# Vahe1994/AQLM

Measured on AMD Instinct MI355X. Metric: QuantizedLinear 1x16g8 matvec algorithmic GB/s (bs=1, Llama-3-8B shapes 4096->4096/11008), higher is better.
Workload: dtype f16; 1 GPU; decode step = 32 blocks x {4096->4096, 4096->11008} 1x16g8 matvec, bs=1, 64 distinct layers (own codes + codebook), 564 MB algorithmic bytes/step, hipGraph replay; scheme=1x16g8, batch=1, kernels=prepacked slice-bucketed gemv (layers of >= 0.5 M codes: both shapes), parallelism=single GPU, packed_bytes=1190264832, canonical_code_bytes=494927872

## Files before the change

aqlm_amd/_native.py:

```python
from __future__ import annotations

import ctypes
import os

_HERE = os.path.dirname(os.path.abspath(__file__))
LIB_PATH = os.environ.get("AQLM_AMD_HIP_LIB") or os.path.join(_HERE, "libaqlm_hip.so")
ABI_VERSION = 9

F16, BF16 = 0, 1
F32 = 2
E_INVALID, E_UNSUPPORTED = -1, -2
MAX_GEMV_BATCH = 8
OP_GEMM_1X16_MFMA = 1
OP_GEMV_1X16_PACKED = 3
OP_GEMV_8X8_LUT = 4
OP_GEMM_KX8_MFMA = 6
OP_GEMV_1X16_G16_PACKED = 5

MAX_SEGMENTS = 4
MAX_ROUTED_PAIRS = 64
MAX_ROUTED_EXPERTS = 256
ROUTED_ENTRY_WORDS = 4
MAX_GROUPED_PAIRS = 1 << 18
GROUPED_TILE_PAIRS = (16, 32, 64, 128)
# ... 219 lines not shown
        raise ImportError(f"{LIB_PATH}: ABI version {v}, expected {ABI_VERSION}; rebuild it")
    return lib


lib = _load()


def last_error() -> str:
    return (lib.aqlm_hip_last_error() or b"").decode("utf-8", "replace")


def check(rc: int, what: str = "") -> None:
    if rc == 0:
        return
    msg = last_error() or what
    if rc == E_UNSUPPORTED:
        raise NotImplementedError(msg)
    if rc == E_INVALID:
        raise ValueError(msg)
    raise AqlmHipError(f"HIP error {rc}: {msg}")


def set_tuning(key: str, value: int) -> None:
    check(lib.aqlm_hip_set_tuning(key.encode(), int(value)), "set_tuning")


def get_tuning(key: str) -> int:
    v = _ci(0)
    check(lib.aqlm_hip_get_tuning(key.encode(), ctypes.byref(v)), "get_tuning")
    return v.value


CAPTURE_OVERLAP_FIELDS = ("seen", "relaxed", "kept_conflict", "kept_window", "runs_broken", "api_failures",
                          "merged", "merge_refused", "nodes_added", "folded")


def capture_overlap_stats(reset: bool = False) -> dict:
    out = (ctypes.c_uint64 * len(CAPTURE_OVERLAP_FIELDS))()
    check(lib.aqlm_hip_capture_overlap_stats_ex(out, len(out)), "capture_overlap_stats")
    if reset:
        check(lib.aqlm_hip_capture_overlap_stats_ex(None, 0), "capture_overlap_stats")
    return dict(zip(CAPTURE_OVERLAP_FIELDS, (int(v) for v in out)))


def packed_image(desc: "PackedDesc", rows: int = 1, dtype: int = F16):
    lds, win = _sz(0), ctypes.c_uint32(0)
    check(lib.aqlm_hip_gemv_1x16_packed_image(ctypes.byref(desc), int(rows), int(dtype), 0, ctypes.byref(lds), ctypes.byref(win), None),
          "packed_image")
    return int(lds.value), int(win.value)


def packed_image_blocks_per_cu(desc: "PackedDesc", rows: int = 1, dtype: int = F16, probe_lds_bytes: int = 0) -> int:
    n = _ci(0)
    check(lib.aqlm_hip_gemv_1x16_packed_image(ctypes.byref(desc), int(rows), int(dtype), int(probe_lds_bytes), None, None, ctypes.byref(n)),
          "packed_image")
    return n.value


def packed_chain_plan(desc: "PackedDesc", next_desc=None, rows: int = 1, dtype: int = F16):
    kept, waves, lds = _ci(0), _ci(0), _sz(0)
    check(lib.aqlm_hip_gemv_1x16_packed_chain_plan(ctypes.byref(desc), int(rows), int(dtype), None if next_desc is None else ctypes.byref(next_desc),
                                                   ctypes.byref(kept), ctypes.byref(waves), ctypes.byref(lds)), "packed_chain_plan")
    return bool(kept.value), int(waves.value), int(lds.value)
```

aqlm_amd/csrc/api.hip:

```cpp
#include <stdarg.h>
#include <string.h>

#include <algorithm>
#include <map>
#include <mutex>
#include <utility>

#include "aqlm_common.h"

namespace aqlm {

static thread_local char g_err[512] = "";

void set_last_error(const char* fmt, ...) {
  va_list ap;
  va_start(ap, fmt);
  vsnprintf(g_err, sizeof(g_err), fmt, ap);
  va_end(ap);
}

int check_hip(hipError_t e, const char* what) {
  if (e == hipSuccess) return 0;
  set_last_error("%s: %s (%d)", what, hipGetErrorString(e), (int)e);
  return (int)e;
// ... 23 lines not shown
static int* tuning_slot(const char* key) {
  Tuning& t = tuning();
  if (!key) return nullptr;
  if (!strcmp(key, "gemv_rows_per_wave")) return &t.gemv_rows_per_wave;
  if (!strcmp(key, "gemv1x16_aux")) return &t.gemv1x16_aux;
  if (!strcmp(key, "gemv1x16_prefetch_cb")) return &t.gemv1x16_prefetch_cb;
  if (!strcmp(key, "kx8_replicas")) return &t.kx8_replicas;
  if (!strcmp(key, "gemm_variant")) return &t.gemm_variant;
  if (!strcmp(key, "kx8_mfma_min_rows")) return &t.kx8_mfma_min_rows;
  if (!strcmp(key, "kx8_xres")) return &t.kx8_xres;
  if (!strcmp(key, "kx8_xres_phased")) return &t.kx8_xres_phased;
  if (!strcmp(key, "kx8_phase_tpb")) return &t.kx8_phase_tpb;
  if (!strcmp(key, "kx8_phase_quads")) return &t.kx8_phase_quads;
  if (!strcmp(key, "kx8_multi_xres_min_rows")) return &t.kx8_multi_xres_min_rows;
  if (!strcmp(key, "kx8_ksplit")) return &t.kx8_ksplit;
  if (!strcmp(key, "kx8_rt")) return &t.kx8_rt;
  if (!strcmp(key, "scan_max_rows")) return &t.scan_max_rows;
  if (!strcmp(key, "scan_prefetch")) return &t.scan_prefetch;
  if (!strcmp(key, "gemm_debug")) return &t.gemm_debug;
  if (!strcmp(key, "gemm_store_nt")) return &t.gemm_store_nt;
  if (!strcmp(key, "force_generic")) return &t.force_generic;
  if (!strcmp(key, "packed_waves")) return &t.packed_waves;
  if (!strcmp(key, "packed_fused_finalize")) return &t.packed_fused_finalize;
  if (!strcmp(key, "packed_prefetch")) return &t.packed_prefetch;
  if (!strcmp(key, "packed_arrange")) return &t.packed_arrange;
  if (!strcmp(key, "packed_xcopies")) return &t.packed_xcopies;
  if (!strcmp(key, "packed_entry_bytes")) return &t.packed_entry_bytes;
  if (!strcmp(key, "packed_debug")) return &t.packed_debug;
  if (!strcmp(key, "packed_fill_rotate")) return &t.packed_fill_rotate;
  if (!strcmp(key, "packed_compact_window")) return &t.packed_compact_window;
  if (!strcmp(key, "packed_capture_window")) return &t.packed_capture_window;
  if (!strcmp(key, "packed_capture_min_run")) return &t.packed_capture_min_run;
  if (!strcmp(key, "packed_capture_merge")) return &t.packed_capture_merge;
  if (!strcmp(key, "packed_group_fold")) return &t.packed_group_fold;
  if (!strcmp(key, "packed_pipe")) return &t.packed_pipe;
  if (!strcmp(key, "packed_prefetch_waves")) return &t.packed_prefetch_waves;
  if (!strcmp(key, "packed_dequant_by_xcd")) return &t.packed_dequant_by_xcd;
  if (!strcmp(key, "lut_waves")) return &t.lut_waves;
  return nullptr;
}

namespace {
struct CaptureOverlapState {
  std::mutex mu;
  capture_overlap::Planner planner;
  uint64_t stats[10] = {0, 0, 0, 0, 0, 0, 0, 0, 0, 0};
  bool off = false;
};
CaptureOverlapState& capture_state() {
  static CaptureOverlapState s;
  return s;
}
hipError_t set_capture_deps(hipStream_t stream, const std::vector<capture_overlap::NodeId>& nodes) {
  static_assert(sizeof(hipGraphNode_t) == sizeof(capture_overlap::NodeId), "a graph node handle is carried as a 64-bit id");
  std::vector<hipGraphNode_t> d;
  for (capture_overlap::NodeId n : nodes) d.push_back(reinterpret_cast<hipGraphNode_t>(static_cast<uintptr_t>(n)));
  return hipStreamUpdateCaptureDependencies(stream, d.empty() ? nullptr : d.data(), d.size(), hipStreamSetCaptureDependencies);
}
bool same_nodes(const std::vector<capture_overlap::NodeId>& a, const std::vector<capture_overlap::NodeId>& b) {
  return a.size() == b.size() && std::is_permutation(a.begin(), a.end(), b.begin());
}
bool read_capture(hipStream_t stream, bool& capturing, unsigned long long& id, std::vector<capture_overlap::NodeId>& deps, hipError_t& err) {
  hipStreamCaptureStatus st = hipStreamCaptureStatusNone;
  const hipGraphNode_t* d = nullptr;
  size_t n = 0;
  hipGraph_t graph = nullptr;
  err = hipStreamGetCaptureInfo_v2(stream, &st, &id, &graph, &d, &n);
  if (err != hipSuccess) return false;
  capturing = st == hipStreamCaptureStatusActive;
  deps.clear();
  if (capturing)
    for (size_t i = 0; i < n; ++i) deps.push_back(static_cast<capture_overlap::NodeId>(reinterpret_cast<uintptr_t>(d[i])));
  return true;
}
}

void CaptureRelax::fail(const char* what, hipError_t e) {
  (void)hipGetLastError();
  CaptureOverlapState& s = capture_state();
  s.off = true;
  ++s.stats[5];
  set_last_error("capture overlap switched off for this process: %s: %s (%d)", what, hipGetErrorString(e), (int)e);
}

CaptureRelax::CaptureRelax(hipStream_t stream) : stream_(stream) {
  if (!stream) return;
  CaptureOverlapState& s = capture_state();
  {
    std::lock_guard<std::mutex> lock(s.mu);
    if (s.off) return;
  }
  bool capturing = false;
  hipError_t err = hipSuccess;
  if (!read_capture(stream, capturing, id_, before_, err)) {
    std::lock_guard<std::mutex> lock(s.mu);
    fail("hipStreamGetCaptureInfo_v2", err);
    return;
  }
  if (!capturing) return;
  const int window = tuning().packed_capture_window;
  std::lock_guard<std::mutex> lock(s.mu);
  ++s.stats[0];
  ++s.stats[8];
  if (window <= 1 && tuning().packed_capture_merge <= 1) ++s.stats[3];
  else active_ = true;
}

void CaptureRelax::apply_plan() {
  CaptureOverlapState& s = capture_state();
  ++s.stats[plan_.kind == capture_overlap::kBroken ? 4 : (int)plan_.kind];
  if (plan_.kind == capture_overlap::kBroken || same_nodes(plan_.deps, before_)) return;
  const hipError_t e = set_capture_deps(stream_, plan_.deps);
  if (e == hipSuccess) {
    changed_ = true;
    return;
  }
  fail("hipStreamUpdateCaptureDependencies", e);
  s.planner.run(id_).reset();
  active_ = false;
}

int CaptureRelax::begin(uint64_t key, const void* member, size_t member_bytes) {
  if (!active_ || begun_) return 0;
  begun_ = true;
  const int merge = std::min(std::max(tuning().packed_capture_merge, 1), capture_overlap::kMaxMerge);
  if (merge > 1 && key != 0 && member) {
    key_ = key;
    member_.assign(static_cast<const unsigned char*>(member), static_cast<const unsigned char*>(member) + member_bytes);
  }
  CaptureOverlapState& s = capture_state();
  std::lock_guard<std::mutex> lock(s.mu);
  plan_ = s.planner.run(id_).plan(before_.data(), before_.size(), fp, tuning().packed_capture_window, tuning().packed_capture_min_run,
                                  key_, merge);
  if (plan_.merge) return plan_.member;
  apply_plan();
  return 0;
}

bool CaptureRelax::join(const hipKernelNodeParams* node, int folded_delta) {
  if (!active_ || !begun_ || done_ || !plan_.merge) return false;
  CaptureOverlapState& s = capture_state();
  std::lock_guard<std::mutex> lock(s.mu);
  capture_overlap::Run& run = s.planner.run(id_);
  const hipError_t e = node && run.latest(plan_)
                           ? hipGraphKernelNodeSetParams(reinterpret_cast<hipGraphNode_t>(static_cast<uintptr_t>(plan_.target)), node)
                           : hipErrorInvalidValue;
  if (e == hipSuccess && run.commit(plan_, plan_.target, fp, member_.data(), member_.size())) {
    ++s.stats[3];
    ++s.stats[6];
    --s.stats[8];
    s.stats[9] += (uint64_t)(int64_t)folded_delta;
    done_ = true;
    return true;
  }
  (void)hipGetLastError();
  ++s.stats[7];
  plan_ = run.plan(before_.data(), before_.size(), fp, tuning().packed_capture_window, tuning().packed_capture_min_run, key_, 1);
  apply_plan();
  return false;
}

int CaptureRelax::launched() {
  if (!active_ || !begun_ || done_) return 0;
  done_ = true;
  CaptureOverlapState& s = capture_state();
  std::lock_guard<std::mutex> lock(s.mu);
  capture_overlap::Run& run = s.planner.run(id_);
  bool capturing = false;
  unsigned long long id = 0;
  std::vector<capture_overlap::NodeId> now;
  hipError_t err = hipSuccess;
  const bool read = read_capture(stream_, capturing, id, now, err);
  std::vector<capture_overlap::NodeId> want;
  if (read && capturing && id == id_ && now.size() == 1 && run.commit(plan_, now[0], std::move(fp), member_.data(), member_.size())) {
    want = run.tail();
  } else {
    if (!read) fail("hipStreamGetCaptureInfo_v2", err);
    run.reset();
    if (!changed_) return 0;
    want = before_;
    for (capture_overlap::NodeId n : now)
      if (std::find(want.begin(), want.end(), n) == want.end()) want.push_back(n);
    if (!read || !capturing) {
      set_last_error("capture overlap: the stream's capture state was lost after a launch that had been moved");
      return AQLM_HIP_E_INVALID;
    }
  }
  if (same_nodes(want, now)) return 0;
  const hipError_t e = set_capture_deps(stream_, want);
  if (e == hipSuccess) return 0;
  run.reset();
  const bool moved = changed_ || want.size() > 1;
  fail("hipStreamUpdateCaptureDependencies", e);
  return moved ? (int)e : 0;
}

CaptureRelax::~CaptureRelax() {
  if (!active_ || !begun_ || done_) return;
  CaptureOverlapState& s = capture_state();
  std::lock_guard<std::mutex> lock(s.mu);
  s.planner.run(id_).reset();
  if (!changed_) return;
  const hipError_t e = set_capture_deps(stream_, before_);
  if (e != hipSuccess) fail("hipStreamUpdateCaptureDependencies", e);
}

__global__ __launch_bounds__(256) void checksum_kernel(const uint8_t* data, size_t bytes, unsigned long long* out) {
  const size_t nwords = (bytes + 3) / 4;
  const bool aligned = (reinterpret_cast<uintptr_t>(data) & 3u) == 0;
  unsigned long long a = 0, b = 0;
  for (size_t i = blockIdx.x * (size_t)256 + threadIdx.x; i < nwords; i += (size_t)gridDim.x * 256) {
    uint32_t w = 0;
    if (aligned && i * 4 + 4 <= bytes) w = reinterpret_cast<const uint32_t*>(data)[i];
    else
      for (size_t k = 0; k < 4 && i * 4 + k < bytes; ++k) w |= (uint32_t)data[i * 4 + k] << (8 * k);
    a += w;
    b += (unsigned long long)w * (((unsigned long long)i * 0x9E3779B97F4A7C15ull) | 1ull);
  }
  for (int o = 32; o > 0; o >>= 1) {
    a += __shfl_xor(a, o, WAVE);
    b += __shfl_xor(b, o, WAVE);
  }
  if ((threadIdx.x & 63) == 0) {
    atomicAdd(&out[0], a);
    atomicAdd(&out[1], b);
  }
}

}

extern "C" int aqlm_hip_checksum(const void* data, size_t bytes, void* out_u64x2, void* stream_) {
  hipStream_t stream = (hipStream_t)stream_;
  if (!out_u64x2 || (!data && bytes) || (reinterpret_cast<uintptr_t>(out_u64x2) & 7u)) {
    aqlm::set_last_error("aqlm_hip_checksum: null pointer argument or misaligned output");
    return AQLM_HIP_E_INVALID;
  }
  if (int e = aqlm::check_hip(hipMemsetAsync(out_u64x2, 0, 16, stream), "checksum memset")) return e;
  if (bytes == 0) return 0;
  const size_t nwords = (bytes + 3) / 4;
  const unsigned blocks = (unsigned)std::min<size_t>(2048, (nwords + 255) / 256);
  hipLaunchKernelGGL(aqlm::checksum_kernel, dim3(blocks), dim3(256), 0, stream, (const uint8_t*)data, bytes, (unsigned long long*)out_u64x2);
  return aqlm::check_hip(hipGetLastError(), "checksum launch");
}

static int capture_overlap_stats(uint64_t* out, int n) {
  aqlm::CaptureOverlapState& s = aqlm::capture_state();
  std::lock_guard<std::mutex> lock(s.mu);
  for (int i = 0; i < 10; ++i) {
    if (!out) s.stats[i] = 0;
    else if (i < n) out[i] = s.stats[i];
  }
  return 0;
}

extern "C" int aqlm_hip_capture_overlap_stats(uint64_t out[6]) { return capture_overlap_stats(out, 6); }

extern "C" int aqlm_hip_capture_overlap_stats_ex(uint64_t* out, int count) {
  if (out && (count < 0 || count > 10)) {
    aqlm::set_last_error("aqlm_hip_capture_overlap_stats_ex: count must be 0..10 (got %d)", count);
    return AQLM_HIP_E_INVALID;
  }
  return capture_overlap_stats(out, count);
}

extern "C" int aqlm_hip_abi_version(void) { return AQLM_HIP_ABI_VERSION; }

extern "C" const char* aqlm_hip_last_error(void) { return aqlm::g_err; }

extern "C" int aqlm_hip_set_tuning(const char* key, int value) {
  int* s = aqlm::tuning_slot(key);
  if (!s) {
    aqlm::set_last_error("aqlm_hip_set_tuning: unknown key '%s'", key ? key : "(null)");
    return AQLM_HIP_E_INVALID;
  }
  *s = value;
  return 0;
}

extern "C" int aqlm_hip_get_tuning(const char* key, int* value) {
  int* s = aqlm::tuning_slot(key);
  if (!s || !value) {
    aqlm::set_last_error("aqlm_hip_get_tuning: unknown key '%s'", key ? key : "(null)");
    return AQLM_HIP_E_INVALID;
  }
  *value = *s;
  return 0;
}
```

aqlm_amd/csrc/aqlm_common.h:

```cpp
#pragma once
#include <hip/hip_runtime.h>
#include <stdint.h>
#include <stdio.h>
#include <string.h>

#include "../../include/aqlm_hip.h"
#include "capture_overlap.h"
#include "group_fold.h"

namespace aqlm {

constexpr int WAVE = 64;

typedef unsigned int u32x4 __attribute__((ext_vector_type(4)));
typedef unsigned int u32x2 __attribute__((ext_vector_type(2)));
typedef _Float16 f16x2 __attribute__((ext_vector_type(2)));
typedef __bf16 bf16x2 __attribute__((ext_vector_type(2)));

constexpr int AUX_DEFAULT = 0;
constexpr int AUX_SC0 = 1;
constexpr int AUX_NT = 2;
constexpr int AUX_SC1 = 16;

struct F16 {
  static constexpr int id = AQLM_HIP_F16;
  static __device__ __forceinline__ float dot2(uint32_t a, uint32_t b, float c) {
    return __builtin_amdgcn_fdot2(__builtin_bit_cast(f16x2, a), __builtin_bit_cast(f16x2, b), c, false);
  }
  static __device__ __forceinline__ float to_float(uint16_t u) { return (float)__builtin_bit_cast(_Float16, u); }
  static __device__ __forceinline__ uint16_t from_float(float f) {
    return __builtin_bit_cast(uint16_t, (_Float16)f);
  }
  static __device__ __forceinline__ float lo(uint32_t a) { return to_float((uint16_t)(a & 0xffffu)); }
  static __device__ __forceinline__ float hi(uint32_t a) { return to_float((uint16_t)(a >> 16)); }
};

struct BF16 {
// ... 89 lines not shown
  int gemv_rows_per_wave = 0;
  int gemv1x16_aux = AUX_DEFAULT;
  int gemv1x16_prefetch_cb = 0;
  int kx8_replicas = 1;
  int gemm_variant = 0;
  int scan_max_rows = 0;
  int scan_prefetch = 4;
  int kx8_xres = 1;
  int kx8_xres_phased = 1;
  int kx8_phase_tpb = 0;
  int kx8_phase_quads = 0;
  int kx8_mfma_min_rows = 2;
  int kx8_multi_xres_min_rows = 2;
  int kx8_ksplit = 0;
  int kx8_rt = 0;
  int gemm_debug = 0;
  int gemm_store_nt = 0;
  int force_generic = 0;
  int packed_fused_finalize = 1;
  int packed_waves = 0;
  int packed_arrange = 1;
  int packed_xcopies = 0;
  int packed_entry_bytes = 0;
  int packed_debug = 0;
  int packed_prefetch = 0;
  int packed_pipe = 1;
  int packed_fill_rotate = 1;
  int packed_compact_window = 0;
  int lut_waves = 0;
  int packed_prefetch_waves = 0;
  int packed_capture_window = capture_overlap::kDefaultWindow;
  int packed_capture_min_run = capture_overlap::kDefaultMinRun;
  int packed_capture_merge = capture_overlap::kDefaultMerge;
  int packed_group_fold = 0;
  int packed_dequant_by_xcd = 1;
};
Tuning& tuning();

class CaptureRelax {
 public:
  explicit CaptureRelax(hipStream_t stream);
  ~CaptureRelax();
  CaptureRelax(const CaptureRelax&) = delete;
  CaptureRelax& operator=(const CaptureRelax&) = delete;
  bool capturing() const { return active_; }
  capture_overlap::Footprint fp;
  int begin(uint64_t key = 0, const void* member = nullptr, size_t member_bytes = 0);
  const std::vector<unsigned char>& group() const { return plan_.payload; }
  bool join(const hipKernelNodeParams* node, int folded_delta = 0);
  int launched();

 private:
  void fail(const char* what, hipError_t e);
  void apply_plan();
  hipStream_t stream_;
  bool active_ = false, begun_ = false, done_ = false, changed_ = false;
  uint64_t key_ = 0;
  std::vector<unsigned char> member_;
  unsigned long long id_ = 0;
  std::vector<capture_overlap::NodeId> before_;
  capture_overlap::Plan plan_;
};

namespace scan {
size_t workspace_bytes(int B, int M, int K);
int run(const void* codes, const void* codebook, const void* scales, const void* bias, const void* X, void* Y, int batch, int out_features,
        int in_features, long xs, long ys, int dtype, void* workspace, hipStream_t stream);
}

inline bool aligned16(const void* p) { return (reinterpret_cast<uintptr_t>(p) & 15u) == 0; }
inline bool aligned8(const void* p) { return (reinterpret_cast<uintptr_t>(p) & 7u) == 0; }
inline bool ids_aligned(const void* ids, int ids_int64) { return (reinterpret_cast<uintptr_t>(ids) & (ids_int64 ? 7u : 3u)) == 0; }

inline int check_not_null(const char* who, bool all_set) {
  if (all_set) return 0;
  set_last_error("%s: null pointer argument", who);
  return AQLM_HIP_E_INVALID;
}
inline int check_aligned(const char* who, const char* what, bool ok) {
  if (ok) return 0;
  set_last_error("%s: %s misaligned", who, what);
  return AQLM_HIP_E_INVALID;
}
inline int check_experts(const char* who, int num_experts, int num_segments) {
  if (num_experts >= 1 && num_experts <= AQLM_HIP_MAX_ROUTED_EXPERTS && num_segments >= 1 && num_segments <= 2) return 0;
  set_last_error("%s: %d experts x %d segments (1..%d x 1..2 supported)", who, num_experts, num_segments, AQLM_HIP_MAX_ROUTED_EXPERTS);
  return AQLM_HIP_E_INVALID;
}
inline int check_pairs(const char* who, int num_pairs, int top_k, int max_pairs) {
// ... 32 lines not shown
```

aqlm_amd/csrc/capture_overlap.h:

```cpp
#ifndef AQLM_CAPTURE_OVERLAP_H_
#define AQLM_CAPTURE_OVERLAP_H_

#include <stddef.h>
#include <stdint.h>

#include <algorithm>
#include <vector>

namespace aqlm {
namespace capture_overlap {

using NodeId = uint64_t;

constexpr int kMaxWindow = 8;
constexpr int kDefaultWindow = 2;
constexpr int kDefaultMinRun = 8;
constexpr int kMaxMerge = 8;
constexpr int kDefaultMerge = 4;
constexpr size_t kMaxRanges = 256;

struct Range {
  uintptr_t begin, end;
  bool writes;
};
// ... 2 lines not shown
  std::vector<Range> ranges;
  void add(const void* p, size_t bytes, bool writes) {
    if (!p || !bytes) return;
    const uintptr_t b = reinterpret_cast<uintptr_t>(p);
    ranges.push_back(Range{b, b + bytes, writes});
  }
  void add_rows(const void* p, int rows, long stride_bytes, size_t row_bytes, bool writes) {
    if (rows > 1 && stride_bytes == (long)row_bytes) return add(p, (size_t)rows * row_bytes, writes);
    for (int r = 0; r < rows; ++r) add(reinterpret_cast<const char*>(p) + (ptrdiff_t)r * stride_bytes, row_bytes, writes);
  }
};

inline bool hazard(const Footprint& a, const Footprint& b) {
  for (const Range& x : a.ranges)
    for (const Range& y : b.ranges)
      if ((x.writes || y.writes) && x.begin < y.end && y.begin < x.end) return true;
  return false;
}

enum Kind { kBroken = 0, kRelaxed = 1, kConflict = 2, kWindow = 3 };

struct Plan {
  Kind kind = kBroken;
  std::vector<NodeId> deps;
  std::vector<size_t> leave;
  bool restart = false;
  uint64_t generation = 0;
  uint64_t key = 0;
  bool merge = false;
  size_t merge_pos = 0;
  NodeId target = 0;
  int member = 0;
  std::vector<unsigned char> payload;
};

class Run {
 public:
  uint64_t capture_id = 0;

  Plan plan(const NodeId* deps, size_t num_deps, const Footprint& fp, int window, int min_run = 1, uint64_t key = 0,
            int merge_max = 1) {
    window = std::min(std::max(window, 1), kMaxWindow);
    merge_max = std::min(merge_max, kMaxMerge);
    Plan p;
    p.key = key;
    p.generation = ++generation_;
    if (!is_tail(deps, num_deps)) {
      p.kind = kBroken;
      p.restart = true;
      p.deps.assign(deps, deps + num_deps);
      return p;
    }
    for (size_t i = 0; i < tail_.size(); ++i)
      if (hazard(tail_[i].fp, fp)) p.leave.push_back(i);
    if (!p.leave.empty()) {
      p.kind = kConflict;
    } else if (length_ < (size_t)std::max(min_run, 1)) {
      p.kind = kWindow;
      for (size_t i = 0; i < tail_.size(); ++i) p.leave.push_back(i);
    } else if ((int)tail_.size() >= window) {
      p.kind = kWindow;
      for (size_t i = 0; key != 0 && i < tail_.size(); ++i) {
        if (tail_[i].key != key || tail_[i].members >= merge_max) continue;
        if (fp.ranges.size() + tail_[i].fp.ranges.size() > kMaxRanges) {
          p.restart = true;
          p.deps.assign(deps, deps + num_deps);
          return p;
        }
        p.merge = true;
        p.merge_pos = i;
        p.target = tail_[i].node;
        p.member = tail_[i].members;
        p.payload = tail_[i].payload;
        return p;
      }
      p.leave.push_back(0);
    } else {
      p.kind = kRelaxed;
      p.deps = base_;
      return p;
    }
    size_t ranges = fp.ranges.size();
    for (size_t i : p.leave) ranges += tail_[i].fp.ranges.size();
    if (ranges > kMaxRanges) {
      p.restart = true;
      p.leave.clear();
      p.deps.assign(deps, deps + num_deps);
      return p;
    }
    for (size_t i : p.leave) p.deps.push_back(tail_[i].node);
    return p;
  }

  bool commit(const Plan& p, NodeId node, Footprint fp, const void* payload = nullptr, size_t payload_bytes = 0) {
    if (p.generation != generation_) return false;
    const unsigned char* pb = static_cast<const unsigned char*>(payload);
    if (p.merge) {
      Entry e = std::move(tail_[p.merge_pos]);
      tail_.erase(tail_.begin() + (ptrdiff_t)p.merge_pos);
      e.node = node;
      e.fp.ranges.insert(e.fp.ranges.end(), fp.ranges.begin(), fp.ranges.end());
      if (pb) e.payload.insert(e.payload.end(), pb, pb + payload_bytes);
      ++e.members;
      ++generation_;
      ++length_;
      tail_.push_back(std::move(e));
      return true;
    }
    if (p.restart) {
      base_ = p.deps;
      tail_.clear();
      length_ = 0;
    } else {
      for (size_t k = p.leave.size(); k-- > 0;) {
        const Footprint& gone = tail_[p.leave[k]].fp;
        fp.ranges.insert(fp.ranges.end(), gone.ranges.begin(), gone.ranges.end());
        tail_.erase(tail_.begin() + (ptrdiff_t)p.leave[k]);
      }
    }
    ++generation_;
    ++length_;
    tail_.push_back(Entry{node, std::move(fp), p.key, 1, std::vector<unsigned char>(pb, pb + (pb ? payload_bytes : 0))});
    return true;
  }

  bool latest(const Plan& p) const { return p.generation == generation_; }

  void reset() {
    ++generation_;
    base_.clear();
    tail_.clear();
    length_ = 0;
  }

  std::vector<NodeId> tail() const {
    std::vector<NodeId> t;
    for (const Entry& e : tail_) t.push_back(e.node);
    return t;
  }
  const std::vector<NodeId>& base() const { return base_; }

 private:
  struct Entry {
    NodeId node;
    Footprint fp;
    uint64_t key;
    int members;
    std::vector<unsigned char> payload;
  };
  bool is_tail(const NodeId* deps, size_t n) const {
    if (tail_.empty() || n != tail_.size()) return false;
    for (size_t i = 0; i < n; ++i) {
      bool found = false;
      for (const Entry& e : tail_) found = found || e.node == deps[i];
      if (!found) return false;
      for (size_t j = 0; j < i; ++j)
        if (deps[j] == deps[i]) return false;
    }
    return true;
  }
  std::vector<NodeId> base_;
  std::vector<Entry> tail_;
  size_t length_ = 0;
  uint64_t generation_ = 0;
};

class Planner {
 public:
  Run& run(uint64_t capture_id) {
    ++clock_;
    size_t lru = 0;
    for (size_t i = 0; i < kSlots; ++i) {
      if (used_[i] && runs_[i].capture_id == capture_id) {
        used_[i] = clock_;
        return runs_[i];
      }
      if (used_[i] < used_[lru]) lru = i;
    }
    runs_[lru].reset();
    runs_[lru].capture_id = capture_id;
    used_[lru] = clock_;
    return runs_[lru];
  }

 private:
  static constexpr size_t kSlots = 4;
  Run runs_[kSlots];
  uint64_t used_[kSlots] = {0, 0, 0, 0};
  uint64_t clock_ = 0;
};

}
}
#endif
```

aqlm_amd/csrc/packed_gemv_entries.h:

```cpp

static bool packed_fused(const aqlm_hip_packed_desc* desc) {
  return tuning().packed_fused_finalize != 0 && desc->codebook_absmax > 0.f && desc->codebook_absmax < __builtin_inff();
}

struct PackedFused {
  const void* scales = nullptr;
  const void* bias = nullptr;
  void* y = nullptr;
  long y_row_stride = 0;
  float cb_absmax = 0.f;
  void* cells = nullptr;
  float* pub = nullptr;
  uint32_t* pub_flag = nullptr;
  uint32_t* pub_epoch = nullptr;
  uint32_t pub_max_elems = 0;
};

struct PackedNext {
  const uint8_t* ent = nullptr;
  const uint8_t* codebook = nullptr;
  uint32_t block_bytes = 0;
};

static chain_hint::Hint packed_chain_hint(const PackedLayout& LN) {
// ... 8 lines not shown
                              long x_row_stride, int dtype, void* workspace, size_t workspace_bytes, hipStream_t stream,
                              const char* who, const PackedFused& fused = PackedFused{}, const PackedNext& next = PackedNext{},
                              CaptureRelax* relax = nullptr) {
  const bool finalizes = fused.y || fused.pub;
  const size_t need = finalizes ? 0 : (size_t)PK_S * nb * L.M * sizeof(float);
  if (need && (!workspace || workspace_bytes < need)) {
    set_last_error("%s: workspace of %zu bytes required, got %zu", who, need, workspace_bytes);
    return AQLM_HIP_E_INVALID;
  }
  const uint8_t* base = (const uint8_t*)packed;
  const uint32_t* ent = (const uint32_t*)(base + L.off_ent);
  const uint32_t* rowstart = (const uint32_t*)(base + L.off_rowstart);
  const uint8_t* cb = L.relabel ? base + L.off_cb : (const uint8_t*)codebook;
  PackedGemvRest rest{};
  rest.winfo = (const uint32_t*)(base + L.off_winfo);
  rest.partial = (float*)workspace;
  rest.x_row_stride = x_row_stride;
  if (finalizes) {
    rest.acc = fused.cells ? (unsigned long long*)fused.cells : (unsigned long long*)(const_cast<uint8_t*>(base) + L.off_acc);
    rest.cb_absmax = fused.cb_absmax;
    rest.scales = (const uint16_t*)fused.scales;
    rest.bias = (const uint16_t*)fused.bias;
    rest.y = (uint16_t*)fused.y;
    rest.y_row_stride = fused.y_row_stride;
  }
#ifdef AQLM_PACKED_TRACE
  rest.trace = workspace && workspace_bytes >= need + (size_t)PK_NST * PK_MAX_NW * 8 * 8 ? (unsigned long long*)((uint8_t*)workspace + need) : nullptr;
  rest.dbg = tuning().packed_debug;
#endif
  int npw = 0;
  if (next.ent && next.codebook && next.block_bytes) npw = packed_chain_waves(L);
  const uint32_t rotate = tuning().packed_fill_rotate ? 1u : 0u;
#if AQLM_PK_G == 8
  auto try_join = [&](bool vg, const PackedGroupSegment& me, unsigned threads, size_t lds, bool& joined) -> int {
    joined = false;
    if (tuning().packed_capture_merge <= 1) {
      if (relax) relax->begin();
      return 0;
    }
    const void* gk = vg ? (dtype == AQLM_HIP_F16 ? (const void*)gemv_1x16_packed_group_kernel<F16, 3, PK_XWIN_COMPACT, 4, true>
                                                 : (const void*)gemv_1x16_packed_group_kernel<BF16, 3, PK_XWIN_COMPACT, 4, true>)
                        : (dtype == AQLM_HIP_F16 ? (const void*)gemv_1x16_packed_group_kernel<F16, 3, PK_XWIN_COMPACT, 4, false>
                                                 : (const void*)gemv_1x16_packed_group_kernel<BF16, 3, PK_XWIN_COMPACT, 4, false>);
    if (int e = ensure_dynamic_lds(gk, lds)) return e;
    const void* fk = vg ? nullptr
                        : (dtype == AQLM_HIP_F16 ? (const void*)gemv_1x16_packed_group_fold_kernel<F16, 3, PK_XWIN_COMPACT, 4>
                                                 : (const void*)gemv_1x16_packed_group_fold_kernel<BF16, 3, PK_XWIN_COMPACT, 4>);
    if (fk)
      if (int e = ensure_dynamic_lds(fk, lds)) return e;
    if (!relax) return 0;
    uint64_t key = (uint64_t)reinterpret_cast<uintptr_t>(gk) * 0x9E3779B97F4A7C15ull ^ ((uint64_t)threads << 32) ^ (uint64_t)lds;
    if (key == 0) key = 1;
    const int n = relax->begin(key, &me, sizeof me);
    if (n <= 0) return 0;
    const std::vector<unsigned char>& members = relax->group();
    if (n >= PK_GROUP_MAX || members.size() != (size_t)n * sizeof(PackedGroupSegment)) {
      relax->join(nullptr);
      return 0;
    }
    PackedGroupParams gp{};
    memcpy(gp.seg, members.data(), members.size());
    gp.seg[n] = me;
    const int key_fold = tuning().packed_group_fold;
    bool one_row_before = fk != nullptr;
    for (int i = 0; i < n; ++i) one_row_before = one_row_before && gp.seg[i].RG <= (int)threads;
    const bool was_folded = one_row_before && group_fold::choose(key_fold, n) > 1;
    int fold = one_row_before && me.RG <= (int)threads ? group_fold::choose(key_fold, n + 1) : 1;
    void* args[2] = {&gp, &fold};
    hipKernelNodeParams node{};
    node.func = const_cast<void*>(fold > 1 ? fk : gk);
    node.gridDim = dim3(group_fold::grid(n + 1, fold));
    node.blockDim = dim3(threads);
    node.sharedMemBytes = (unsigned)lds;
    node.kernelParams = args;
    node.extra = nullptr;
    joined = relax->join(&node, (fold > 1 ? 1 : 0) - (was_folded ? 1 : 0));
    return 0;
  };
#endif
  auto launch = [&](auto kern, auto lds_map) -> int {
    const size_t lds = decltype(lds_map)::total(L.in_groups, L.RG, npw, L.NW);
    if (lds > 160 * 1024) { npw = 0; }
    const size_t lds_final = decltype(lds_map)::total(L.in_groups, L.RG, npw, L.NW);
    if (int e = ensure_dynamic_lds(reinterpret_cast<const void*>(kern), lds_final)) return e;
    PackedGemvRest r = rest;
    r.pub = fused.pub;
    r.pub_flag = fused.pub_flag;
    r.pub_epoch = fused.pub_epoch;
    r.pub_max_elems = fused.pub_max_elems;
    if (npw) {
      r.next_ent = next.ent;
      r.next_codebook = next.codebook;
      r.next_block_bytes = next.block_bytes;
    }
    bool joined = false;
#if AQLM_PK_G == 8
    if (decltype(lds_map)::TIGHT && nb == 1 && npw == 0 && fused.y && !fused.pub) {
      PackedGroupSegment me{};
      me.codebook = cb;
      me.x = x;
      me.ent = ent;
      me.rowstart = rowstart;
      me.in_groups = L.in_groups;
      me.RG = L.RG;
      me.M = L.M;
      me.geom = (uint32_t)L.NW | ((uint32_t)L.XC << 8) | (rotate << 15) | ((uint32_t)L.T << 16);
      me.ent_bytes = (uint32_t)L.ent_bytes;
      me.rest = r;
      if (int e = try_join(false, me, (unsigned)L.NW * 64u, lds_final, joined)) return e;
    } else
#endif
    if (relax) relax->begin();
    if (joined) return 0;
    hipLaunchKernelGGL(kern, dim3(PK_NST), dim3((L.NW + npw) * 64), lds_final, stream, cb, x, ent, rowstart, L.in_groups,
                       (uint32_t)L.NW | ((uint32_t)L.XC << 8) | ((uint32_t)npw << 12) | (rotate << 15) | ((uint32_t)L.T << 16), L.RG,
                       (uint32_t)L.ent_bytes, L.M, r);
    return check_hip(hipGetLastError(), "gemv_1x16_packed launch");
  };
  const bool sf = nb == 1 && packed_b1_slice_first(L.in_groups, L.RG);
  const bool compact = nb == 1 && packed_b1_compact(L, packed_b1_pd(L));
#if AQLM_PK_G == 8
  if (L.G.vg) {
    if (fused.pub != nullptr || L.EB != 4) {
      set_last_error("%s: a variable-geometry buffer runs on the single-layer matvec entries only (repack with "
                     "AQLM_HIP_PREPACK_UNIFORM_ONLY for the publish form)", who);
      return AQLM_HIP_E_UNSUPPORTED;
    }
    uint32_t ns[4] = {0u, 0u, 0u, 0u};
    for (int i = 0; i < PK_S; ++i) ns[i >> 2] |= (uint32_t)L.G.first[i] << ((i & 3) * 8);
    auto launch_vg = [&](auto kern, auto lds_map) -> int {
      const size_t lds = decltype(lds_map)::total(L.in_groups, L.RG, 0, L.NW);
      if (int e = ensure_dynamic_lds(reinterpret_cast<const void*>(kern), lds)) return e;
      bool joined = false;
      if (decltype(lds_map)::TIGHT && nb == 1 && fused.y) {
        PackedGroupSegment me{};
        me.codebook = cb;
        me.x = x;
        me.ent = ent;
        me.rowstart = rowstart;
        me.in_groups = L.in_groups;
        me.RG = L.RG;
        me.M = L.M;
        me.geom = (uint32_t)L.NW | ((uint32_t)L.XC << 8) | (rotate << 15) | ((uint32_t)L.T << 16);
        me.ent_bytes = (uint32_t)PK_NST * (uint32_t)L.NW * (uint32_t)L.T * 1024u;
        for (int i = 0; i < 4; ++i) me.ns[i] = ns[i];
        me.rest = rest;
        if (int e = try_join(true, me, (unsigned)L.NW * 64u, lds, joined)) return e;
      } else if (relax) {
        relax->begin();
      }
      if (joined) return 0;
      hipLaunchKernelGGL(kern, dim3(PK_NST), dim3(L.NW * 64), lds, stream, cb, x, ent, (uint32_t)(L.off_ent - L.off_rowstart),
                         (uint32_t)L.in_groups | ((uint32_t)L.RG << 12), (uint32_t)L.NW | ((uint32_t)L.XC << 8) | (rotate << 15) | ((uint32_t)L.T << 16),
                         L.M, ns[0], ns[1], ns[2], ns[3], rest);
      return check_hip(hipGetLastError(), "gemv_1x16_packed (variable geometry) launch");
    };
    return dispatch_packed_vg(dtype, nb, sf, compact, launch_vg);
  }
#endif
  if (fused.pub != nullptr) return dispatch_packed<PublishKernels>(dtype, nb, pick_pd(L), L.EB, sf, false, launch);
  return dispatch_packed<SingleKernels>(dtype, nb, pick_pd(L), L.EB, sf, compact, launch);
}

static int packed_check_args(const char* who, const aqlm_hip_packed_desc* desc, const void* packed, const void* codebook,
                             const void* x, int batch, long x_row_stride, int dtype, PackedLayout& L, int& max_b) {
  if (!packed || !codebook || !x || !desc) {
    set_last_error("%s: null pointer argument", who);
    return AQLM_HIP_E_INVALID;
  }
  if (dtype != AQLM_HIP_F16 && dtype != AQLM_HIP_BF16) {
    set_last_error("%s: AQLM HIP kernels only support float16 and bfloat16 (dtype id %d)", who, dtype);
    return AQLM_HIP_E_UNSUPPORTED;
  }
  if (!desc_layout(desc, L)) {
    set_last_error("%s: invalid packed descriptor", who);
    return AQLM_HIP_E_INVALID;
  }
  if (batch < 1 || batch > AQLM_HIP_MAX_GEMV_BATCH || !aligned16(packed) || !aligned16(codebook) || !aligned16(x) ||
      (batch > 1 && x_row_stride % 8 != 0)) {
    set_last_error("%s: batch must be 1..%d and packed / codebook / x rows 16-B aligned (batch %d)", who,
                   AQLM_HIP_MAX_GEMV_BATCH, batch);
    return AQLM_HIP_E_INVALID;
  }
  if (L.relabel && !(desc->flags & AQLM_HIP_PACKED_HAS_CODEBOOK)) {
    set_last_error("%s: a relabelled buffer needs its codebook image: call aqlm_hip_packed_set_codebook first (and again whenever "
                   "the codebook changes)", who);
    return AQLM_HIP_E_INVALID;
// ... 459 lines not shown
```

Before: 1925 GB/s.

## Regroup run-head launches into merged group kernel nodes during graph capture

During hipGraph capture, the first launches of an overlap run (before the minimum run length is reached) were kept as separate kernel nodes. They are now recorded with their full launch description and, once the run qualifies, regrouped: same-key launches are rewritten into multi-segment group (or folded) kernel nodes, the surplus nodes are destroyed, and the stream dependencies are reset. The aim is to cut the number of kernel nodes and their launch overhead at run heads in the replayed graph. This adds graph-surgery complexity with a fallback that disables head regrouping on any API error, and it is on by default through a new tuning key.

```diff
diff --git a/aqlm_amd/_native.py b/aqlm_amd/_native.py
--- a/aqlm_amd/_native.py
+++ b/aqlm_amd/_native.py
@@ -275,7 +275,7 @@
 
 
 CAPTURE_OVERLAP_FIELDS = ("seen", "relaxed", "kept_conflict", "kept_window", "runs_broken", "api_failures",
-                          "merged", "merge_refused", "nodes_added", "folded")
+                          "merged", "merge_refused", "nodes_added", "folded", "head_regrouped", "head_moved", "head_refused")
 
 
 def capture_overlap_stats(reset: bool = False) -> dict:
diff --git a/aqlm_amd/csrc/api.hip b/aqlm_amd/csrc/api.hip
--- a/aqlm_amd/csrc/api.hip
+++ b/aqlm_amd/csrc/api.hip
@@ -79,6 +79,7 @@
   if (!strcmp(key, "packed_capture_window")) return &t.packed_capture_window;
   if (!strcmp(key, "packed_capture_min_run")) return &t.packed_capture_min_run;
   if (!strcmp(key, "packed_capture_merge")) return &t.packed_capture_merge;
+  if (!strcmp(key, "packed_capture_head")) return &t.packed_capture_head;
   if (!strcmp(key, "packed_group_fold")) return &t.packed_group_fold;
   if (!strcmp(key, "packed_pipe")) return &t.packed_pipe;
   if (!strcmp(key, "packed_prefetch_waves")) return &t.packed_prefetch_waves;
@@ -91,8 +92,10 @@
 struct CaptureOverlapState {
   std::mutex mu;
   capture_overlap::Planner planner;
-  uint64_t stats[10] = {0, 0, 0, 0, 0, 0, 0, 0, 0, 0};
+  static constexpr int kStats = 13;
+  uint64_t stats[kStats] = {0, 0, 0, 0, 0, 0, 0, 0, 0, 0, 0, 0, 0};
   bool off = false;
+  bool head_off = false;
 };
 CaptureOverlapState& capture_state() {
   static CaptureOverlapState s;
@@ -122,6 +125,48 @@
 }
 }
 
+bool capture_build_node(const unsigned char* members, int n, CaptureNode& out) {
+  if (!members || n < 1 || n > capture_overlap::kMaxMerge) return false;
+  CaptureMember m0;
+  memcpy(&m0, members, sizeof m0);
+  out.params = hipKernelNodeParams{};
+  out.params.blockDim = dim3(m0.threads);
+  out.params.sharedMemBytes = m0.lds;
+  out.params.kernelParams = out.args;
+  out.params.extra = nullptr;
+  out.fold = 1;
+  if (n == 1) {
+    if (!m0.func || m0.nargs == 0 || m0.nargs > CaptureMember::kMaxArgs) return false;
+    out.store.assign(m0.args, m0.args + CaptureMember::kArgBytes);
+    for (unsigned i = 0; i < m0.nargs; ++i) {
+      if (m0.arg_off[i] >= CaptureMember::kArgBytes) return false;
+      out.args[i] = out.store.data() + m0.arg_off[i];
+    }
+    out.params.func = const_cast<void*>(m0.func);
+    out.params.gridDim = dim3(m0.grid);
+    return true;
+  }
+  if (!m0.group_func || m0.seg_bytes == 0 || m0.seg_bytes > CaptureMember::kSegBytes || m0.seg_bytes % 8 != 0) return false;
+  const size_t segs = (size_t)capture_overlap::kMaxMerge * m0.seg_bytes;
+  out.store.assign(segs + sizeof(int), 0);
+  bool one_row = m0.fold_func != nullptr;
+  for (int i = 0; i < n; ++i) {
+    CaptureMember m;
+    memcpy(&m, members + (size_t)i * sizeof m, sizeof m);
+    if (m.group_func != m0.group_func || m.fold_func != m0.fold_func || m.threads != m0.threads || m.lds != m0.lds || m.seg_bytes != m0.seg_bytes)
+      return false;
+    memcpy(out.store.data() + (size_t)i * m0.seg_bytes, m.seg, m0.seg_bytes);
+    one_row = one_row && m.rows_per_group <= (int)m0.threads;
+  }
+  out.fold = one_row ? group_fold::choose(tuning().packed_group_fold, n) : 1;
+  memcpy(out.store.data() + segs, &out.fold, sizeof(int));
+  out.args[0] = out.store.data();
+  out.args[1] = out.store.data() + segs;
+  out.params.func = const_cast<void*>(out.fold > 1 ? m0.fold_func : m0.group_func);
+  out.params.gridDim = dim3(group_fold::grid(n, out.fold));
+  return true;
+}
+
 void CaptureRelax::fail(const char* what, hipError_t e) {
   (void)hipGetLastError();
   CaptureOverlapState& s = capture_state();
@@ -171,10 +216,8 @@
   if (!active_ || begun_) return 0;
   begun_ = true;
   const int merge = std::min(std::max(tuning().packed_capture_merge, 1), capture_overlap::kMaxMerge);
-  if (merge > 1 && key != 0 && member) {
-    key_ = key;
-    member_.assign(static_cast<const unsigned char*>(member), static_cast<const unsigned char*>(member) + member_bytes);
-  }
+  if (member) member_.assign(static_cast<const unsigned char*>(member), static_cast<const unsigned char*>(member) + member_bytes);
+  if (merge > 1 && key != 0 && member) key_ = key;
   CaptureOverlapState& s = capture_state();
   std::lock_guard<std::mutex> lock(s.mu);
   plan_ = s.planner.run(id_).plan(before_.data(), before_.size(), fp, tuning().packed_capture_window, tuning().packed_capture_min_run,
@@ -207,6 +250,72 @@
   return false;
 }
 
+bool CaptureRelax::join_members() {
+  const size_t n = plan_.merge ? (size_t)plan_.member : 0;
+  if (n == 0 || n >= (size_t)capture_overlap::kMaxMerge || plan_.payload.size() != n * sizeof(CaptureMember) || member_.size() != sizeof(CaptureMember))
+    return join(nullptr);
+  std::vector<unsigned char> all(plan_.payload);
+  all.insert(all.end(), member_.begin(), member_.end());
+  CaptureNode before, after;
+  if (!capture_build_node(all.data(), (int)n + 1, after)) return join(nullptr);
+  const bool was_folded = capture_build_node(plan_.payload.data(), (int)n, before) && before.fold > 1;
+  return join(&after.params, (after.fold > 1 ? 1 : 0) - (was_folded ? 1 : 0));
+}
+
+void CaptureRelax::regroup_head(capture_overlap::Run& run, std::vector<capture_overlap::NodeId>& now) {
+  CaptureOverlapState& s = capture_state();
+  if (s.head_off || tuning().packed_capture_head == 0) return;
+  const int merge = std::min(std::max(tuning().packed_capture_merge, 1), capture_overlap::kMaxMerge);
+  const capture_overlap::HeadScript script = run.regroup_head(tuning().packed_capture_min_run, merge);
+  if (script.empty()) return;
+  using capture_overlap::HeadStep;
+  std::vector<CaptureNode> nodes(script.steps.size());
+  uint64_t folded = 0;
+  for (size_t k = 0; k < script.steps.size(); ++k) {
+    const HeadStep& st = script.steps[k];
+    if (st.op != HeadStep::kRewrite) continue;
+    if (st.payload.size() != st.members.size() * sizeof(CaptureMember) ||
+        !capture_build_node(st.payload.data(), (int)st.members.size(), nodes[k])) {
+      run.head_applied(0);
+      ++s.stats[12];
+      return;
+    }
+    folded += nodes[k].fold > 1;
+  }
+  size_t done = 0;
+  hipError_t e = hipSuccess;
+  const char* what = "";
+  for (; done < script.steps.size(); ++done) {
+    const HeadStep& st = script.steps[done];
+    const hipGraphNode_t node = reinterpret_cast<hipGraphNode_t>(static_cast<uintptr_t>(st.node));
+    if (st.op == HeadStep::kRewrite) {
+      what = "hipGraphKernelNodeSetParams";
+      e = hipGraphKernelNodeSetParams(node, &nodes[done].params);
+    } else if (st.op == HeadStep::kSetStreamDeps) {
+      what = "hipStreamUpdateCaptureDependencies";
+      e = set_capture_deps(stream_, {st.node});
+      if (e == hipSuccess) now.assign(1, st.node);
+    } else {
+      what = "hipGraphDestroyNode";
+      e = hipGraphDestroyNode(node);
+    }
+    if (e != hipSuccess) break;
+    head_touched_ = true;
+  }
+  run.head_applied(done);
+  if (done == script.steps.size()) {
+    ++s.stats[10];
+    s.stats[11] += script.moved;
+    s.stats[9] += folded;
+    return;
+  }
+  (void)hipGetLastError();
+  ++s.stats[12];
+  s.head_off = true;
+  set_last_error("capture overlap: regrouping of run heads switched off for this process: %s: %s (%d) at step %zu of %zu", what,
+                 hipGetErrorString(e), (int)e, done, script.steps.size());
+}
+
 int CaptureRelax::launched() {
   if (!active_ || !begun_ || done_) return 0;
   done_ = true;
@@ -220,6 +329,7 @@
   const bool read = read_capture(stream_, capturing, id, now, err);
   std::vector<capture_overlap::NodeId> want;
   if (read && capturing && id == id_ && now.size() == 1 && run.commit(plan_, now[0], std::move(fp), member_.data(), member_.size())) {
+    if (plan_.head) regroup_head(run, now);
     want = run.tail();
   } else {
     if (!read) fail("hipStreamGetCaptureInfo_v2", err);
@@ -237,7 +347,7 @@
   const hipError_t e = set_capture_deps(stream_, want);
   if (e == hipSuccess) return 0;
   run.reset();
-  const bool moved = changed_ || want.size() > 1;
+  const bool moved = changed_ || head_touched_ || want.size() > 1;
   fail("hipStreamUpdateCaptureDependencies", e);
   return moved ? (int)e : 0;
 }
@@ -293,7 +403,7 @@
 static int capture_overlap_stats(uint64_t* out, int n) {
   aqlm::CaptureOverlapState& s = aqlm::capture_state();
   std::lock_guard<std::mutex> lock(s.mu);
-  for (int i = 0; i < 10; ++i) {
+  for (int i = 0; i < aqlm::CaptureOverlapState::kStats; ++i) {
     if (!out) s.stats[i] = 0;
     else if (i < n) out[i] = s.stats[i];
   }
@@ -303,8 +413,8 @@
 extern "C" int aqlm_hip_capture_overlap_stats(uint64_t out[6]) { return capture_overlap_stats(out, 6); }
 
 extern "C" int aqlm_hip_capture_overlap_stats_ex(uint64_t* out, int count) {
-  if (out && (count < 0 || count > 10)) {
-    aqlm::set_last_error("aqlm_hip_capture_overlap_stats_ex: count must be 0..10 (got %d)", count);
+  if (out && (count < 0 || count > aqlm::CaptureOverlapState::kStats)) {
+    aqlm::set_last_error("aqlm_hip_capture_overlap_stats_ex: count must be 0..13 (got %d)", count);
     return AQLM_HIP_E_INVALID;
   }
   return capture_overlap_stats(out, count);
diff --git a/aqlm_amd/csrc/aqlm_common.h b/aqlm_amd/csrc/aqlm_common.h
--- a/aqlm_amd/csrc/aqlm_common.h
+++ b/aqlm_amd/csrc/aqlm_common.h
@@ -3,6 +3,9 @@
 #include <stdint.h>
 #include <stdio.h>
 #include <string.h>
+
+#include <type_traits>
+#include <vector>
 
 #include "../../include/aqlm_hip.h"
 #include "capture_overlap.h"
@@ -158,10 +161,55 @@
   int packed_capture_window = capture_overlap::kDefaultWindow;
   int packed_capture_min_run = capture_overlap::kDefaultMinRun;
   int packed_capture_merge = capture_overlap::kDefaultMerge;
+  int packed_capture_head = 1;
   int packed_group_fold = 0;
   int packed_dequant_by_xcd = 1;
 };
 Tuning& tuning();
+
+struct CaptureMember {
+  static constexpr unsigned kMaxArgs = 12, kArgBytes = 320, kSegBytes = 256;
+  const void* func;
+  unsigned grid, threads, lds, nargs;
+  uint16_t arg_off[kMaxArgs];
+  const void* group_func;
+  const void* fold_func;
+  unsigned seg_bytes;
+  int rows_per_group;
+  alignas(8) unsigned char args[kArgBytes];
+  alignas(8) unsigned char seg[kSegBytes];
+};
+template <class... P, class... A>
+inline bool capture_member_launch(CaptureMember& m, void (*kern)(P...), unsigned grid, unsigned threads, size_t lds, const A&... a) {
+  static_assert(sizeof...(P) == sizeof...(A) && sizeof...(P) <= CaptureMember::kMaxArgs, "one value per kernel parameter");
+  m.func = reinterpret_cast<const void*>(kern);
+  m.grid = grid;
+  m.threads = threads;
+  m.lds = (unsigned)lds;
+  m.nargs = 0;
+  size_t at = 0;
+  bool fits = true;
+  auto put = [&](const auto& v) {
+    static_assert(alignof(decltype(v)) <= 8, "arguments are packed at 8-byte boundaries");
+    at = (at + 7) & ~(size_t)7;
+    if (at + sizeof v > CaptureMember::kArgBytes) {
+      fits = false;
+      return;
+    }
+    memcpy(m.args + at, &v, sizeof v);
+    m.arg_off[m.nargs++] = (uint16_t)at;
+    at += sizeof v;
+  };
+  (put(static_cast<std::remove_cv_t<P>>(a)), ...);
+  return fits;
+}
+struct CaptureNode {
+  hipKernelNodeParams params;
+  int fold = 1;
+  void* args[CaptureMember::kMaxArgs];
+  std::vector<unsigned char> store;
+};
+bool capture_build_node(const unsigned char* members, int n, CaptureNode& out);
 
 class CaptureRelax {
  public:
@@ -174,13 +222,15 @@
   int begin(uint64_t key = 0, const void* member = nullptr, size_t member_bytes = 0);
   const std::vector<unsigned char>& group() const { return plan_.payload; }
   bool join(const hipKernelNodeParams* node, int folded_delta = 0);
+  bool join_members();
   int launched();
 
  private:
   void fail(const char* what, hipError_t e);
   void apply_plan();
+  void regroup_head(capture_overlap::Run& run, std::vector<capture_overlap::NodeId>& now);
   hipStream_t stream_;
-  bool active_ = false, begun_ = false, done_ = false, changed_ = false;
+  bool active_ = false, begun_ = false, done_ = false, changed_ = false, head_touched_ = false;
   uint64_t key_ = 0;
   std::vector<unsigned char> member_;
   unsigned long long id_ = 0;
diff --git a/aqlm_amd/csrc/capture_overlap.h b/aqlm_amd/csrc/capture_overlap.h
--- a/aqlm_amd/csrc/capture_overlap.h
+++ b/aqlm_amd/csrc/capture_overlap.h
@@ -58,6 +58,22 @@
   NodeId target = 0;
   int member = 0;
   std::vector<unsigned char> payload;
+  bool head = false;
+};
+
+struct HeadStep {
+  enum Op { kRewrite = 0, kSetStreamDeps = 1, kDestroy = 2 };
+  Op op = kRewrite;
+  NodeId node = 0;
+  uint64_t key = 0;
+  std::vector<size_t> members;
+  std::vector<unsigned char> payload;
+};
+struct HeadScript {
+  std::vector<HeadStep> steps;
+  size_t groups = 0;
+  size_t moved = 0;
+  bool empty() const { return steps.empty(); }
 };
 
 class Run {
@@ -71,12 +87,14 @@
     Plan p;
     p.key = key;
     p.generation = ++generation_;
+    p.head = true;
     if (!is_tail(deps, num_deps)) {
       p.kind = kBroken;
       p.restart = true;
       p.deps.assign(deps, deps + num_deps);
       return p;
     }
+    p.head = length_ < (size_t)std::max(min_run, 1);
     for (size_t i = 0; i < tail_.size(); ++i)
       if (hazard(tail_[i].fp, fp)) p.leave.push_back(i);
     if (!p.leave.empty()) {
@@ -90,6 +108,7 @@
         if (tail_[i].key != key || tail_[i].members >= merge_max) continue;
         if (fp.ranges.size() + tail_[i].fp.ranges.size() > kMaxRanges) {
           p.restart = true;
+          p.head = true;
           p.deps.assign(deps, deps + num_deps);
           return p;
         }
@@ -110,6 +129,7 @@
     for (size_t i : p.leave) ranges += tail_[i].fp.ranges.size();
     if (ranges > kMaxRanges) {
       p.restart = true;
+      p.head = true;
       p.leave.clear();
       p.deps.assign(deps, deps + num_deps);
       return p;
@@ -131,12 +151,17 @@
       ++generation_;
       ++length_;
       tail_.push_back(std::move(e));
+      head_.clear();
       return true;
     }
+    Footprint own;
+    if (p.head && head_.size() == (p.restart ? 0 : length_)) own = fp;
     if (p.restart) {
       base_ = p.deps;
       tail_.clear();
       length_ = 0;
+      head_.clear();
+      head_ok_ = p.kind == kBroken;
     } else {
       for (size_t k = p.leave.size(); k-- > 0;) {
         const Footprint& gone = tail_[p.leave[k]].fp;
@@ -144,10 +169,92 @@
         tail_.erase(tail_.begin() + (ptrdiff_t)p.leave[k]);
       }
     }
+    if (p.head && head_.size() == length_) {
+      if (p.kind == kConflict) head_ok_ = false;
+      head_.push_back(HeadLaunch{node, own, p.key, std::vector<unsigned char>(pb, pb + (pb ? payload_bytes : 0))});
+    } else {
+      head_.clear();
+    }
     ++generation_;
     ++length_;
     tail_.push_back(Entry{node, std::move(fp), p.key, 1, std::vector<unsigned char>(pb, pb + (pb ? payload_bytes : 0))});
     return true;
+  }
+
+  HeadScript regroup_head(int min_run, int merge_max) {
+    HeadScript s;
+    merge_max = std::min(merge_max, kMaxMerge);
+    const size_t n = head_.size();
+    if (length_ < (size_t)std::max(min_run, 1)) return s;
+    if (!head_ok_ || merge_max <= 1 || n < 2 || n != length_ || n != (size_t)std::max(min_run, 1) || tail_.size() != 1 ||
+        tail_[0].node != head_[n - 1].node) {
+      head_.clear();
+      return s;
+    }
+    std::vector<std::vector<size_t>> groups;
+    for (size_t i = 0; i < n; ++i) {
+      size_t g = groups.size();
+      for (size_t k = 0; head_[i].key != 0 && k < groups.size() && g == groups.size(); ++k)
+        if (head_[groups[k][0]].key == head_[i].key && groups[k].size() < (size_t)merge_max) g = k;
+      if (g == groups.size()) groups.emplace_back();
+      groups[g].push_back(i);
+    }
+    bool possible = groups.size() < n;
+    for (size_t g = 0; g < groups.size(); ++g)
+      for (size_t i : groups[g])
+        if (i != g && head_[i].payload.empty()) possible = false;
+    if (!possible) {
+      head_.clear();
+      return s;
+    }
+    for (size_t g = 0; g < groups.size(); ++g) {
+      if (groups[g].size() == 1 && groups[g][0] == g) continue;
+      HeadStep st;
+      st.op = HeadStep::kRewrite;
+      st.node = head_[g].node;
+      st.key = head_[groups[g][0]].key;
+      st.members = groups[g];
+      for (size_t i : groups[g]) st.payload.insert(st.payload.end(), head_[i].payload.begin(), head_[i].payload.end());
+      s.steps.push_back(std::move(st));
+    }
+    for (size_t j = n; j-- > groups.size();) {
+      HeadStep dep, gone;
+      dep.op = HeadStep::kSetStreamDeps;
+      dep.node = head_[j - 1].node;
+      gone.op = HeadStep::kDestroy;
+      gone.node = head_[j].node;
+      s.steps.push_back(std::move(dep));
+      s.steps.push_back(std::move(gone));
+    }
+    s.groups = groups.size();
+    s.moved = n - groups.size();
+    pending_ = s;
+    pending_last_ = std::move(groups.back());
+    ++generation_;
+    return s;
+  }
+
+  void head_applied(size_t steps_done) {
+    if (pending_.empty() || tail_.size() != 1 || head_.empty()) return;
+    ++generation_;
+    Entry& e = tail_[0];
+    if (steps_done >= pending_.steps.size()) {
+      e.node = head_[pending_.groups - 1].node;
+      e.key = head_[pending_last_[0]].key;
+      e.members = (int)pending_last_.size();
+      e.payload.clear();
+      for (size_t i : pending_last_) e.payload.insert(e.payload.end(), head_[i].payload.begin(), head_[i].payload.end());
+    } else {
+      size_t destroyed = 0;
+      for (size_t k = 0; k < steps_done; ++k) destroyed += pending_.steps[k].op == HeadStep::kDestroy;
+      e.node = head_[head_.size() - 1 - destroyed].node;
+      e.key = 0;
+      e.members = 1;
+      e.payload.clear();
+    }
+    pending_ = HeadScript{};
+    pending_last_.clear();
+    head_.clear();
   }
 
   bool latest(const Plan& p) const { return p.generation == generation_; }
@@ -157,6 +264,10 @@
     base_.clear();
     tail_.clear();
     length_ = 0;
+    head_.clear();
+    head_ok_ = false;
+    pending_ = HeadScript{};
+    pending_last_.clear();
   }
 
   std::vector<NodeId> tail() const {
@@ -185,8 +296,18 @@
     }
     return true;
   }
+  struct HeadLaunch {
+    NodeId node;
+    Footprint fp;
+    uint64_t key;
+    std::vector<unsigned char> payload;
+  };
   std::vector<NodeId> base_;
   std::vector<Entry> tail_;
+  std::vector<HeadLaunch> head_;
+  bool head_ok_ = false;
+  HeadScript pending_;
+  std::vector<size_t> pending_last_;
   size_t length_ = 0;
   uint64_t generation_ = 0;
 };
diff --git a/aqlm_amd/csrc/packed_gemv_entries.h b/aqlm_amd/csrc/packed_gemv_entries.h
--- a/aqlm_amd/csrc/packed_gemv_entries.h
+++ b/aqlm_amd/csrc/packed_gemv_entries.h
@@ -64,10 +64,13 @@
   if (next.ent && next.codebook && next.block_bytes) npw = packed_chain_waves(L);
   const uint32_t rotate = tuning().packed_fill_rotate ? 1u : 0u;
 #if AQLM_PK_G == 8
-  auto try_join = [&](bool vg, const PackedGroupSegment& me, unsigned threads, size_t lds, bool& joined) -> int {
+  static_assert(sizeof(PackedGroupSegment) <= CaptureMember::kSegBytes && sizeof(PackedGroupSegment) % 8 == 0 &&
+                    sizeof(PackedGroupParams) == (size_t)capture_overlap::kMaxMerge * sizeof(PackedGroupSegment),
+                "capture_build_node lays the segments out as PackedGroupParams");
+  auto try_join = [&](bool vg, const PackedGroupSegment& me, unsigned threads, size_t lds, CaptureMember& member, bool& joined) -> int {
     joined = false;
     if (tuning().packed_capture_merge <= 1) {
-      if (relax) relax->begin();
+      if (relax) relax->begin(0, member.func ? &member : nullptr, sizeof member);
       return 0;
     }
     const void* gk = vg ? (dtype == AQLM_HIP_F16 ? (const void*)gemv_1x16_packed_group_kernel<F16, 3, PK_XWIN_COMPACT, 4, true>
@@ -83,30 +86,12 @@
     if (!relax) return 0;
     uint64_t key = (uint64_t)reinterpret_cast<uintptr_t>(gk) * 0x9E3779B97F4A7C15ull ^ ((uint64_t)threads << 32) ^ (uint64_t)lds;
     if (key == 0) key = 1;
-    const int n = relax->begin(key, &me, sizeof me);
-    if (n <= 0) return 0;
-    const std::vector<unsigned char>& members = relax->group();
-    if (n >= PK_GROUP_MAX || members.size() != (size_t)n * sizeof(PackedGroupSegment)) {
-      relax->join(nullptr);
-      return 0;
-    }
-    PackedGroupParams gp{};
-    memcpy(gp.seg, members.data(), members.size());
-    gp.seg[n] = me;
-    const int key_fold = tuning().packed_group_fold;
-    bool one_row_before = fk != nullptr;
-    for (int i = 0; i < n; ++i) one_row_before = one_row_before && gp.seg[i].RG <= (int)threads;
-    const bool was_folded = one_row_before && group_fold::choose(key_fold, n) > 1;
-    int fold = one_row_before && me.RG <= (int)threads ? group_fold::choose(key_fold, n + 1) : 1;
-    void* args[2] = {&gp, &fold};
-    hipKernelNodeParams node{};
-    node.func = const_cast<void*>(fold > 1 ? fk : gk);
-    node.gridDim = dim3(group_fold::grid(n + 1, fold));
-    node.blockDim = dim3(threads);
-    node.sharedMemBytes = (unsigned)lds;
-    node.kernelParams = args;
-    node.extra = nullptr;
-    joined = relax->join(&node, (fold > 1 ? 1 : 0) - (was_folded ? 1 : 0));
+    member.group_func = gk;
+    member.fold_func = fk;
+    member.seg_bytes = (unsigned)sizeof me;
+    member.rows_per_group = me.RG;
+    memcpy(member.seg, &me, sizeof me);
+    if (relax->begin(key, &member, sizeof member) > 0) joined = relax->join_members();
     return 0;
   };
 #endif
@@ -126,6 +111,11 @@
       r.next_block_bytes = next.block_bytes;
     }
     bool joined = false;
+    const uint32_t geom = (uint32_t)L.NW | ((uint32_t)L.XC << 8) | ((uint32_t)npw << 12) | (rotate << 15) | ((uint32_t)L.T << 16);
+    CaptureMember member{};
+    const bool described = relax && relax->capturing() &&
+                           capture_member_launch(member, kern, (unsigned)PK_NST, (unsigned)(L.NW + npw) * 64u, lds_final, cb, x, ent, rowstart,
+                                                 L.in_groups, geom, L.RG, (uint32_t)L.ent_bytes, L.M, r);
 #if AQLM_PK_G == 8
     if (decltype(lds_map)::TIGHT && nb == 1 && npw == 0 && fused.y && !fused.pub) {
       PackedGroupSegment me{};
@@ -139,13 +129,12 @@
       me.geom = (uint32_t)L.NW | ((uint32_t)L.XC << 8) | (rotate << 15) | ((uint32_t)L.T << 16);
       me.ent_bytes = (uint32_t)L.ent_bytes;
       me.rest = r;
-      if (int e = try_join(false, me, (unsigned)L.NW * 64u, lds_final, joined)) return e;
+      if (int e = try_join(false, me, (unsigned)L.NW * 64u, lds_final, member, joined)) return e;
     } else
 #endif
-    if (relax) relax->begin();
+    if (relax) relax->begin(0, described ? &member : nullptr, sizeof member);
     if (joined) return 0;
-    hipLaunchKernelGGL(kern, dim3(PK_NST), dim3((L.NW + npw) * 64), lds_final, stream, cb, x, ent, rowstart, L.in_groups,
-                       (uint32_t)L.NW | ((uint32_t)L.XC << 8) | ((uint32_t)npw << 12) | (rotate << 15) | ((uint32_t)L.T << 16), L.RG,
+    hipLaunchKernelGGL(kern, dim3(PK_NST), dim3((L.NW + npw) * 64), lds_final, stream, cb, x, ent, rowstart, L.in_groups, geom, L.RG,
                        (uint32_t)L.ent_bytes, L.M, r);
     return check_hip(hipGetLastError(), "gemv_1x16_packed launch");
   };
@@ -164,6 +153,12 @@
       const size_t lds = decltype(lds_map)::total(L.in_groups, L.RG, 0, L.NW);
       if (int e = ensure_dynamic_lds(reinterpret_cast<const void*>(kern), lds)) return e;
       bool joined = false;
+      const uint32_t geom = (uint32_t)L.NW | ((uint32_t)L.XC << 8) | (rotate << 15) | ((uint32_t)L.T << 16);
+      CaptureMember member{};
+      const bool described = relax && relax->capturing() &&
+                             capture_member_launch(member, kern, (unsigned)PK_NST, (unsigned)L.NW * 64u, lds, cb, x, ent,
+                                                   (uint32_t)(L.off_ent - L.off_rowstart), (uint32_t)L.in_groups | ((uint32_t)L.RG << 12), geom, L.M,
+                                                   ns[0], ns[1], ns[2], ns[3], rest);
       if (decltype(lds_map)::TIGHT && nb == 1 && fused.y) {
         PackedGroupSegment me{};
         me.codebook = cb;
@@ -177,14 +172,13 @@
         me.ent_bytes = (uint32_t)PK_NST * (uint32_t)L.NW * (uint32_t)L.T * 1024u;
         for (int i = 0; i < 4; ++i) me.ns[i] = ns[i];
         me.rest = rest;
-        if (int e = try_join(true, me, (unsigned)L.NW * 64u, lds, joined)) return e;
+        if (int e = try_join(true, me, (unsigned)L.NW * 64u, lds, member, joined)) return e;
       } else if (relax) {
-        relax->begin();
+        relax->begin(0, described ? &member : nullptr, sizeof member);
       }
       if (joined) return 0;
       hipLaunchKernelGGL(kern, dim3(PK_NST), dim3(L.NW * 64), lds, stream, cb, x, ent, (uint32_t)(L.off_ent - L.off_rowstart),
-                         (uint32_t)L.in_groups | ((uint32_t)L.RG << 12), (uint32_t)L.NW | ((uint32_t)L.XC << 8) | (rotate << 15) | ((uint32_t)L.T << 16),
-                         L.M, ns[0], ns[1], ns[2], ns[3], rest);
+                         (uint32_t)L.in_groups | ((uint32_t)L.RG << 12), geom, L.M, ns[0], ns[1], ns[2], ns[3], rest);
       return check_hip(hipGetLastError(), "gemv_1x16_packed (variable geometry) launch");
     };
     return dispatch_packed_vg(dtype, nb, sf, compact, launch_vg);
```

Measured after the change: 2088 GB/s (median of 6 runs). 8.5% higher.
